# yutongwangBIT/multi_orbslam3

Hardware: AMD Instinct MI355X
Metric: tracking+localBA frames/sec (aggregate over agents; 1 agent per GPU) (higher is better)
Workload: dtype u8/int32 (ORB front-end, Hamming), f64 (local BA)

## Files before the change

multi_orbslam3_amd/csrc/lba.hip:

```cpp

#include <time.h>

#include <condition_variable>
#include <atomic>
#include <unistd.h>
#include <mutex>
#include <thread>

#include "common.hpp"
#include "wave.hpp"

#include <algorithm>
#include <cmath>
#include <limits>
#include <numeric>
#include <type_traits>

using namespace orbg;

#include "ldlt_mfma.hpp"
#include "ldlt_xcd.hpp"
#include "se3.hpp"
#include "lm_driver.hpp"

// ... 544 lines not shown
                                               const double* __restrict__ points, CamT c, Huber hb, double* __restrict__ err,
                                               double* __restrict__ chi2, const int* __restrict__ pose_col,
                                               const int* __restrict__ point_col, double* __restrict__ EB,
                                               const int* __restrict__ ps_start, const int* __restrict__ ps_edges,
                                               double* __restrict__ Hpp, double* __restrict__ bp, double* __restrict__ partial,
                                               unsigned* __restrict__ ticket, const double* __restrict__ scale_partial, int n_scale_partial,
                                               const int* __restrict__ ok_flag, HostRec* __restrict__ rec, unsigned seq, int n_edge_blocks,
                                               int nL, const int* __restrict__ pt_start, const int* __restrict__ pt_edges,
                                               double* __restrict__ Hll, double* __restrict__ bl, LmIn lm) {
  const int bid = (int)blockIdx.x;
  LBA_PROF_BEGIN(0);
  if (bid < nP) {
    lin_poses_block<true>(bid, ps_start, ps_edges, edges, poses, points, c, hb, err, chi2, Hpp, bp);
  } else if (bid < nP + n_edge_blocks) {
    linearize_block<true>(bid - nP, n_edges, edges, poses, points, c, hb, err, chi2, pose_col, point_col, EB,
                          TrialPublish{partial, ticket, scale_partial, n_scale_partial, ok_flag, rec, seq, n_edge_blocks, lm});
  } else if (bid - nP - n_edge_blocks < errlin_point_blocks(nL)) {
    lin_points_block(bid - nP - n_edge_blocks, nL, pt_start, pt_edges, edges, poses, points, c, hb, Hll, bl);
  } else {
    publish_trial_when_all_arrived(n_edge_blocks, partial, ticket, scale_partial, n_scale_partial, ok_flag, rec, seq, lm);
  }
  LBA_PROF_END();
}


__global__ __launch_bounds__(256) void k_reduce_points(int nL, const int* __restrict__ pt_start, const int* __restrict__ pt_edges,
                                                      const double* __restrict__ EB, double* __restrict__ Hll, double* __restrict__ bl) {
  const int l = blockIdx.x * 256 + threadIdx.x;
  if (l >= nL) return;
  double acc[9];
#pragma unroll
  for (int i = 0; i < 9; i++) acc[i] = 0;
  const int jb = pt_start[l], je = pt_start[l + 1];
  double part[4][9];
#pragma unroll
  for (int q = 0; q < 4; q++)
#pragma unroll
    for (int i = 0; i < 9; i++) part[q][i] = 0;
  for (int j0 = jb; j0 < je; j0 += 4) {
    int id[4];
#pragma unroll
    for (int q = 0; q < 4; q++) id[q] = pt_edges[min(j0 + q, je - 1)];
    double v[4][9];
#pragma unroll
    for (int q = 0; q < 4; q++) {
      const double* eb = EB + (size_t)id[q] * kEB + 18;
#pragma unroll
      for (int i = 0; i < 9; i++) v[q][i] = eb[i];
    }
#pragma unroll
    for (int q = 0; q < 4; q++)
      if (j0 + q < je) {
#pragma unroll
        for (int i = 0; i < 9; i++) part[q][i] += v[q][i];
      }
  }
#pragma unroll
  for (int i = 0; i < 9; i++) acc[i] = ((part[0][i] + part[1][i]) + part[2][i]) + part[3][i];
  for (int i = 0; i < 6; i++) Hll[6 * (size_t)l + i] = acc[i];
  for (int i = 0; i < 3; i++) bl[3 * (size_t)l + i] = acc[6 + i];
}

__device__ inline void inv3_sym(const double* h6, double lambda, double* o) {
  const double m0 = h6[0] + lambda, m1 = h6[1], m2 = h6[2], m4 = h6[3] + lambda, m5 = h6[4], m8 = h6[5] + lambda;
  const double c00 = m4 * m8 - m5 * m5, c01 = m5 * m2 - m1 * m8, c02 = m1 * m5 - m4 * m2;
  const double det = m0 * c00 + m1 * c01 + m2 * c02;
  const double id = 1.0 / det;
  o[0] = c00 * id; o[1] = c01 * id; o[2] = c02 * id;
  o[3] = o[1]; o[4] = (m0 * m8 - m2 * m2) * id; o[5] = (m2 * m1 - m0 * m5) * id;
  o[6] = o[2]; o[7] = o[5]; o[8] = (m0 * m4 - m1 * m1) * id;
}

struct PairItem { int ea, eb, l; };

constexpr int kSchurThreads = 256;

constexpr int kSortPfThreads = 64, kSortPfCap = 64;
template <int NT, int CAP, bool BY_EDGE = false>
__device__ __forceinline__ void sort_pf_block(int bid, int nL, const int* __restrict__ pf_start, int* __restrict__ pf_edges,
                                              int* __restrict__ pf_col, unsigned long long* __restrict__ lm_mask,
                                              const lba_edge* __restrict__ edges, const int* __restrict__ pose_col) {
  __shared__ int s_e[NT][CAP + 1];
  __shared__ int s_c[NT][CAP + 1];
  const int l = bid * NT + threadIdx.x;
  if (l >= nL) return;
  const int b0 = pf_start[l], cnt = pf_start[l + 1] - b0;
  unsigned long long m = 0;
  if (cnt <= CAP) {
    int* const se = s_e[threadIdx.x];
    int* const sc = s_c[threadIdx.x];
    for (int j = 0; j < cnt; j++) se[j] = pf_edges[b0 + j];
    for (int j = 0; j < cnt; j++) sc[j] = pose_col[edges[se[j]].pose];
    for (int a2 = 1; a2 < cnt; a2++) {
      const int e = se[a2], key = sc[a2];
      int b2 = a2 - 1;
      while (b2 >= 0 && (sc[b2] > key || (BY_EDGE && sc[b2] == key && se[b2] > e))) { se[b2 + 1] = se[b2]; sc[b2 + 1] = sc[b2]; b2--; }
      se[b2 + 1] = e; sc[b2 + 1] = key;
    }
    for (int j = 0; j < cnt; j++) { pf_edges[b0 + j] = se[j]; pf_col[b0 + j] = sc[j]; m |= 1ull << sc[j]; }
  } else {
    for (int a2 = b0 + 1; a2 < b0 + cnt; a2++) {
      const int e = pf_edges[a2], key = pose_col[edges[e].pose];
      int b2 = a2 - 1;
      while (b2 >= b0 && (pose_col[edges[pf_edges[b2]].pose] > key ||
                          (BY_EDGE && pose_col[edges[pf_edges[b2]].pose] == key && pf_edges[b2] > e))) { pf_edges[b2 + 1] = pf_edges[b2]; b2--; }
      pf_edges[b2 + 1] = e;
    }
    for (int j = b0; j < b0 + cnt; j++) { const int c = pose_col[edges[pf_edges[j]].pose]; pf_col[j] = c; m |= 1ull << c; }
  }
  lm_mask[l] = m;
}

__global__ __launch_bounds__(256) void k_csr_fill(int n_edges, const lba_edge* __restrict__ edges, const int* __restrict__ pose_col,
                                                 const int* __restrict__ point_col, int* __restrict__ cur_pt, int* __restrict__ cur_ps,
                                                 int* __restrict__ cur_pf, int* __restrict__ pt_edges, int* __restrict__ ps_edges,
                                                 int* __restrict__ pf_edges) {
  __shared__ int s_cnt[64], s_base[64];
  const int k = blockIdx.x * 256 + threadIdx.x;
  if (threadIdx.x < 64) s_cnt[threadIdx.x] = 0;
  __syncthreads();
  int lc = -1, pc = -1, my = 0;
  if (k < n_edges) {
    const lba_edge e = edges[k];
    lc = point_col[e.point]; pc = pose_col[e.pose];
    pt_edges[atomicAdd(&cur_pt[lc], 1)] = k;
    if (pc >= 0) { pf_edges[atomicAdd(&cur_pf[lc], 1)] = k; my = atomicAdd(&s_cnt[pc], 1); }
  }
  __syncthreads();
  if (threadIdx.x < 64 && s_cnt[threadIdx.x] > 0) s_base[threadIdx.x] = atomicAdd(&cur_ps[threadIdx.x], s_cnt[threadIdx.x]);
  __syncthreads();
  if (pc >= 0) ps_edges[s_base[pc] + my] = k;
}
constexpr int kPrep256Cap = 16, kPrep256Pad = 8, kPrep256Zero = 4;
constexpr int kCsrPoseCap = 4096, kCsrPtCap = 16;
__global__ __launch_bounds__(256) void k_csr_sort(int nP, int nL, const int* __restrict__ ps_start, int* __restrict__ ps_edges,
                                                 const int* __restrict__ pt_start, int* __restrict__ pt_edges,
                                                 const int* __restrict__ pf_start, int* __restrict__ pf_edges, int* __restrict__ pf_col,
                                                 unsigned long long* __restrict__ lm_mask, const lba_edge* __restrict__ edges,
                                                 const int* __restrict__ pose_col, int n_unknowns, double* __restrict__ St,
                                                 double* __restrict__ xzero, int n_zero) {
  __shared__ int s_pose[kCsrPoseCap];
  __shared__ int s_pt[256][kCsrPtCap + 1];
  int bid = (int)blockIdx.x;
  const int tid = threadIdx.x;
  if (bid < nP) {
    const int b0 = ps_start[bid], cnt = ps_start[bid + 1] - b0;
    int m = 1;
    while (m < cnt) m <<= 1;
    for (int i = tid; i < m; i += 256) s_pose[i] = i < cnt ? ps_edges[b0 + i] : 0x7FFFFFFF;
    __syncthreads();
    for (int k2 = 2; k2 <= m; k2 <<= 1)
      for (int j = k2 >> 1; j > 0; j >>= 1) {
        for (int i = tid; i < m; i += 256) {
          const int ixj = i ^ j;
          if (ixj > i) {
            const int a = s_pose[i], c = s_pose[ixj];
            const bool up = (i & k2) == 0;
            if ((a > c) == up) { s_pose[i] = c; s_pose[ixj] = a; }
          }
        }
        __syncthreads();
      }
    for (int i = tid; i < cnt; i += 256) ps_edges[b0 + i] = s_pose[i];
    return;
  }
  bid -= nP;
  const int n_pt_blocks = (nL + 255) / 256;
  if (bid < n_pt_blocks) {
    const int l = bid * 256 + tid;
    if (l < nL) {
      const int b0 = pt_start[l], cnt = pt_start[l + 1] - b0;
      if (cnt <= kCsrPtCap) {
        int* const se = s_pt[tid];
        for (int j = 0; j < cnt; j++) se[j] = pt_edges[b0 + j];
        for (int a2 = 1; a2 < cnt; a2++) {
          const int e = se[a2];
          int b2 = a2 - 1;
          while (b2 >= 0 && se[b2] > e) { se[b2 + 1] = se[b2]; b2--; }
          se[b2 + 1] = e;
        }
        for (int j = 0; j < cnt; j++) pt_edges[b0 + j] = se[j];
      } else {
        for (int a2 = b0 + 1; a2 < b0 + cnt; a2++) {
          const int e = pt_edges[a2];
          int b2 = a2 - 1;
          while (b2 >= b0 && pt_edges[b2] > e) { pt_edges[b2 + 1] = pt_edges[b2]; b2--; }
          pt_edges[b2 + 1] = e;
        }
      }
    }
    sort_pf_block<256, kCsrPtCap, true>(bid, nL, pf_start, pf_edges, pf_col, lm_mask, edges, pose_col);
    return;
  }
  bid -= n_pt_blocks;
  if (bid < kPrep256Pad) { if (St) ldltm::image_pad_range(n_unknowns, St, bid * 256 + tid, kPrep256Pad * 256); return; }
  bid -= kPrep256Pad;
  for (int i = bid * 256 + tid; i < n_zero; i += kPrep256Zero * 256) xzero[i] = 0.0;
}

template <class CamT>
__global__ __launch_bounds__(256) void k_errlin_prep(int n_errlin_blocks, int n_sort_blocks, int* __restrict__ pf_edges_w, int* __restrict__ pf_col_w,
                                                    const int* __restrict__ pf_start, unsigned long long* __restrict__ lm_mask,
                                                    int n_unknowns, double* __restrict__ St, double* __restrict__ xzero, int n_zero,
                                                    int nP, int n_edges, const lba_edge* __restrict__ edges, const PoseQ* __restrict__ poses,
                                               const double* __restrict__ points, CamT c, Huber hb, double* __restrict__ err,
                                               double* __restrict__ chi2, const int* __restrict__ pose_col,
                                               const int* __restrict__ point_col, double* __restrict__ EB,
                                               const int* __restrict__ ps_start, const int* __restrict__ ps_edges,
                                               double* __restrict__ Hpp, double* __restrict__ bp, double* __restrict__ partial,
                                               unsigned* __restrict__ ticket, const double* __restrict__ scale_partial, int n_scale_partial,
                                               const int* __restrict__ ok_flag, HostRec* __restrict__ rec, unsigned seq, int n_edge_blocks,
                                               int nL, const int* __restrict__ pt_start, const int* __restrict__ pt_edges,
                                               double* __restrict__ Hll, double* __restrict__ bl, LmIn lm) {
  int bid = (int)blockIdx.x;
  if (bid >= n_errlin_blocks) {
    bid -= n_errlin_blocks;
    if (bid < n_sort_blocks) { sort_pf_block<256, kPrep256Cap>(bid, nL, pf_start, pf_edges_w, pf_col_w, lm_mask, edges, pose_col); return; }
    bid -= n_sort_blocks;
    if (bid < kPrep256Pad) { if (St) ldltm::image_pad_range(n_unknowns, St, bid * 256 + (int)threadIdx.x, kPrep256Pad * 256); return; }
    bid -= kPrep256Pad;
    for (int i = bid * 256 + (int)threadIdx.x; i < n_zero; i += kPrep256Zero * 256) xzero[i] = 0.0;
    return;
  }

  
  if (bid < nP) {
    lin_poses_block<true>(bid, ps_start, ps_edges, edges, poses, points, c, hb, err, chi2, Hpp, bp);
  } else if (bid < nP + n_edge_blocks) {
    linearize_block<true>(bid - nP, n_edges, edges, poses, points, c, hb, err, chi2, pose_col, point_col, EB,
                          TrialPublish{partial, ticket, scale_partial, n_scale_partial, ok_flag, rec, seq, n_edge_blocks, lm});
  } else if (bid - nP - n_edge_blocks < errlin_point_blocks(nL)) {
    lin_points_block(bid - nP - n_edge_blocks, nL, pt_start, pt_edges, edges, poses, points, c, hb, Hll, bl);
  } else {
    publish_trial_when_all_arrived(n_edge_blocks, partial, ticket, scale_partial, n_scale_partial, ok_flag, rec, seq, lm);
  }
}

__global__ __launch_bounds__(kSortPfThreads) void k_prep(int n_sort_blocks, int nL, const int* __restrict__ pf_start, int* __restrict__ pf_edges,
                                                        int* __restrict__ pf_col, unsigned long long* __restrict__ lm_mask,
                                                        const lba_edge* __restrict__ edges, const int* __restrict__ pose_col,
                                                        int n, double* __restrict__ St, double* __restrict__ xzero, int n_zero) {
  constexpr int kPadBlocks = 32;
  const int bid = (int)blockIdx.x;
  if (bid < n_sort_blocks) { sort_pf_block<kSortPfThreads, kSortPfCap>(bid, nL, pf_start, pf_edges, pf_col, lm_mask, edges, pose_col); return; }
  if (bid < n_sort_blocks + kPadBlocks) {
    if (St) ldltm::image_pad_range(n, St, (bid - n_sort_blocks) * kSortPfThreads + (int)threadIdx.x, kPadBlocks * kSortPfThreads);
    return;
  }
  const int nz = (int)gridDim.x - n_sort_blocks - kPadBlocks;
  for (int i = (bid - n_sort_blocks - kPadBlocks) * kSortPfThreads + (int)threadIdx.x; i < n_zero; i += nz * kSortPfThreads) xzero[i] = 0.0;
}

__device__ __forceinline__ void build_items_block(int pr, int nP, int nL, const unsigned long long* __restrict__ lm_mask,
                                                  const int* __restrict__ pf_start, const int* __restrict__ pf_edges,
                                                  const int* __restrict__ pf_col, PairItem* __restrict__ items, int cap,
                                                  int* __restrict__ pair_count) {
  __shared__ int wcount[4];
  const int tid = threadIdx.x, lane = tid & 63, wv = tid >> 6;
  int i1 = 0, rem = pr;
  while (rem >= nP - i1) { rem -= nP - i1; i1++; }
  const int i2 = i1 + rem;
  const unsigned long long need = (1ull << i1) | (1ull << i2);
  PairItem* out = items + (size_t)pr * cap;
  int running = 0;
  for (int l0 = 0; l0 < nL; l0 += 256) {
    const int l = l0 + tid;
    const unsigned long long m = l < nL ? lm_mask[l] : 0ull;
    const bool has = (m & need) == need;
    const unsigned long long bal = __ballot(has);
    if (lane == 0) wcount[wv] = __popcll(bal);
    __syncthreads();
    int before = 0, total = 0;
#pragma unroll
    for (int w = 0; w < 4; w++) { const int c = wcount[w]; if (w < wv) before += c; total += c; }
    if (has) {
      const int pos = running + before + __popcll(bal & ((1ull << lane) - 1ull));
      const int b0 = pf_start[l];
      const int ea = pf_edges[b0 + __popcll(m & ((1ull << i1) - 1ull))];
      const int eb = pf_edges[b0 + __popcll(m & ((1ull << i2) - 1ull))];
      if (pos < cap) out[pos] = PairItem{ea, eb, l};
    }
    running += total;
    __syncthreads();
  }
  if (tid == 0) pair_count[pr] = min(running, cap);
}
__global__ __launch_bounds__(256) void k_build_items(int nP, int nL, const unsigned long long* __restrict__ lm_mask,
                                                    const int* __restrict__ pf_start, const int* __restrict__ pf_edges,
                                                    const int* __restrict__ pf_col, PairItem* __restrict__ items, int cap,
                                                    int* __restrict__ pair_count) {
  build_items_block((int)blockIdx.x, nP, nL, lm_mask, pf_start, pf_edges, pf_col, items, cap, pair_count);
}

template <int PASSES>
__global__ __launch_bounds__(kSchurThreads) void k_schur(int nP, const int* __restrict__ pair_i1, const int* __restrict__ pair_i2,
                                                        const int* __restrict__ pair_start, const PairItem* __restrict__ items,
                                                        const double* __restrict__ EB, const double* __restrict__ Hll,
                                                        const double* __restrict__ bl, const double* __restrict__ Hpp,
                                                        const double* __restrict__ bp, double lambda_v, double* __restrict__ S,
                                                        double* __restrict__ bs, const double* __restrict__ lambda_p, int item_cap,
                                                        const int* __restrict__ pair_count, double* __restrict__ St) {
  const double lambda = lambda_p ? *lambda_p : lambda_v;
  constexpr int kSeg = 65, kRow = 4 * kSeg + 1, kPass = 42 / PASSES;
  __shared__ double red[kPass * kRow];
  __shared__ double part[42][4];
  LBA_PROF_BEGIN(1);
  int pr;
  {
    const int nb = gridDim.x, q = nb >> 3, r = nb & 7, k = blockIdx.x & 7;
    pr = k * q + min(k, r) + (blockIdx.x >> 3);
  }
  int i1, i2;
  if (pair_i1) { i1 = pair_i1[pr]; i2 = pair_i2[pr]; }
  else {
    int rem = pr; i1 = 0;
    while (rem >= nP - i1) { rem -= nP - i1; i1++; }
    i2 = i1 + rem;
  }
  const int tid = threadIdx.x;
  double acc[36], cacc[6];
#pragma unroll
  for (int i = 0; i < 36; i++) acc[i] = 0;
#pragma unroll
  for (int i = 0; i < 6; i++) cacc[i] = 0;
  const bool diag = i1 == i2;
  const int j0 = pair_start ? pair_start[pr] : pr * item_cap;
  const int j1 = pair_start ? pair_start[pr + 1] : j0 + pair_count[pr];
  for (int j = j0 + tid; j < j1; j += kSchurThreads) {
    const PairItem it = items[j];
    double Dinv[9];
    inv3_sym(Hll + 6 * (size_t)it.l, lambda, Dinv);
    const double* Bi = EB + (size_t)it.ea * kEB;
    const double* Bj = EB + (size_t)it.eb * kEB;
    double BD[18];
#pragma unroll
    for (int a = 0; a < 6; a++)
#pragma unroll
      for (int c = 0; c < 3; c++) BD[3 * a + c] = Bi[3 * a] * Dinv[c] + Bi[3 * a + 1] * Dinv[3 + c] + Bi[3 * a + 2] * Dinv[6 + c];
#pragma unroll
    for (int a = 0; a < 6; a++)
#pragma unroll
      for (int c = 0; c < 6; c++) acc[6 * a + c] += BD[3 * a] * Bj[3 * c] + BD[3 * a + 1] * Bj[3 * c + 1] + BD[3 * a + 2] * Bj[3 * c + 2];
    if (diag) {
      const double* b = bl + 3 * (size_t)it.l;
#pragma unroll
      for (int a = 0; a < 6; a++) cacc[a] += BD[3 * a] * b[0] + BD[3 * a + 1] * b[1] + BD[3 * a + 2] * b[2];
    }
  }
  LBA_PROF_PHASE(0, 0);
  const int slot = (tid >> 6) * kSeg + (tid & 63);
  const int nval = diag ? 42 : 36;
#pragma unroll
  for (int ps = 0; ps < PASSES; ps++) {
    if (ps == 1) __syncthreads();
#pragma unroll
    for (int i = 0; i < kPass; i++) {
      const int v = ps * kPass + i;
      red[i * kRow + slot] = v < 36 ? acc[v < 36 ? v : 0] : cacc[v >= 36 ? v - 36 : 0];
    }
    __syncthreads();
    if (tid < 4 * kPass && ps * kPass + (tid >> 2) < nval) {
      const int o = tid >> 2, q = tid & 3;
      const double* r = red + o * kRow + q * kSeg;
      double s = 0;
#pragma unroll
      for (int k0 = 0; k0 < 64; k0 += 16) {
        double v[16];
#pragma unroll
        for (int u = 0; u < 16; u++) v[u] = r[k0 + u];
#pragma unroll
        for (int u = 0; u < 16; u++) s += v[u];
      }
      part[ps * kPass + o][q] = s;
    }
  }
  __syncthreads();
  LBA_PROF_PHASE(0, 1);
  const int n = 6 * nP;
  if (tid < 36) {
    const double s = ((part[tid][0] + part[tid][1]) + part[tid][2]) + part[tid][3];
    const int a = tid / 6, c = tid % 6;
    double v = -s;
    if (diag) {
      const int lo = a < c ? a : c, hi = a < c ? c : a;
      const int u = lo * 6 - lo * (lo - 1) / 2 + (hi - lo);
      v += Hpp[21 * (size_t)i1 + u] + (a == c ? lambda : 0.0);
    }
    if (St) {
      const int r = 6 * i1 + a, cc = 6 * i2 + c;
      const int p0 = ldltm::tile_image_pos(r, cc), p1 = ldltm::tile_image_pos(cc, r);
      if (p0 >= 0) St[p0] = v;
      if (p1 >= 0 && r != cc) St[p1] = v;
    } else {
      S[(size_t)(6 * i1 + a) * n + 6 * i2 + c] = v;
      if (!diag) S[(size_t)(6 * i2 + c) * n + 6 * i1 + a] = v;
    }
  } else if (diag && tid < 42) {
    const int a = tid - 36;
    const double s = ((part[tid][0] + part[tid][1]) + part[tid][2]) + part[tid][3];
    const double v = bp[6 * (size_t)i1 + a] - s;
    bs[6 * i1 + a] = v;
    if (St) ldltm::image_put_rhs(St, n, 6 * i1 + a, v);
  }
  LBA_PROF_END();
}

#include "ldlt_wide.hpp"

template <int NT>
__global__ __launch_bounds__(NT) void k_update(int n_poses, int n_points, int nP, const int* __restrict__ pose_col,
                                               const int* __restrict__ point_col, const PoseQ* __restrict__ poses,
                                               const double* __restrict__ points, double* __restrict__ x,
                                               const int* __restrict__ pf_start, const int* __restrict__ pf_edges,
                                               const int* __restrict__ pf_col, const double* __restrict__ EB,
                                               const double* __restrict__ Hll, const double* __restrict__ bl, double lambda_v,
                                               PoseQ* __restrict__ poses_out, double* __restrict__ points_out,
                                               const double* __restrict__ bp, double* __restrict__ scale_partial,
                                               const double* __restrict__ lambda_p) {
  LBA_PROF_BEGIN(2);
  const double lambda = lambda_p ? *lambda_p : lambda_v;
  __shared__ double red[NT];
  const int i = blockIdx.x * NT + threadIdx.x;
  double sc = 0;
  if (i < n_points) {
    const int l = point_col[i];
    double dx[3] = {0, 0, 0};
    if (l >= 0) {
      double cl[3] = {bl[3 * (size_t)l], bl[3 * (size_t)l + 1], bl[3 * (size_t)l + 2]};
      constexpr int kUpdChunk = 8;
      const int j1 = pf_start[l + 1];
      for (int j0 = pf_start[l]; j0 < j1; j0 += kUpdChunk) {
        int eid[kUpdChunk], col[kUpdChunk];
#pragma unroll
        for (int u = 0; u < kUpdChunk; u++) { const int j = min(j0 + u, j1 - 1); eid[u] = pf_edges[j]; col[u] = pf_col[j]; }
        double Bv[kUpdChunk][18], xv[kUpdChunk][6];
#pragma unroll
        for (int u = 0; u < kUpdChunk; u++) {
          const double* Bi = EB + (size_t)eid[u] * kEB;
          const double* xp = x + 6 * (size_t)col[u];
#pragma unroll
          for (int q = 0; q < 18; q++) Bv[u][q] = Bi[q];
#pragma unroll
          for (int a = 0; a < 6; a++) xv[u][a] = xp[a];
        }
#pragma unroll
        for (int u = 0; u < kUpdChunk; u++)
          if (j0 + u < j1) {
#pragma unroll
            for (int c = 0; c < 3; c++)
#pragma unroll
              for (int a = 0; a < 6; a++) cl[c] -= Bv[u][3 * a + c] * xv[u][a];
          }
      }
      double Dinv[9];
      inv3_sym(Hll + 6 * (size_t)l, lambda, Dinv);
      for (int a = 0; a < 3; a++) {
        dx[a] = Dinv[3 * a] * cl[0] + Dinv[3 * a + 1] * cl[1] + Dinv[3 * a + 2] * cl[2];
        x[6 * (size_t)nP + 3 * (size_t)l + a] = dx[a];
        sc += dx[a] * (lambda * dx[a] + bl[3 * (size_t)l + a]);
      }
    }
    for (int a = 0; a < 3; a++) points_out[3 * (size_t)i + a] = points[3 * (size_t)i + a] + dx[a];
  } else if (i < n_points + n_poses) {
    const int p = i - n_points;
    const int c = pose_col[p];
    if (c >= 0) {
      pose_oplus(poses[p], x + 6 * (size_t)c, &poses_out[p]);
      for (int a = 0; a < 6; a++) { const double xv = x[6 * (size_t)c + a]; sc += xv * (lambda * xv + bp[6 * (size_t)c + a]); }
    } else {
      poses_out[p] = poses[p];
    }
  }
  LBA_PROF_PHASE(0, 0);
  red[threadIdx.x] = sc;
  __syncthreads();
  for (int s2 = NT / 2; s2 > 0; s2 >>= 1) {
    if ((int)threadIdx.x < s2) red[threadIdx.x] += red[threadIdx.x + s2];
    __syncthreads();
  }
  if (threadIdx.x == 0) scale_partial[blockIdx.x] = red[0];
  LBA_PROF_END();
}

__device__ __forceinline__ void finish_block(int n_partial, const double* __restrict__ partial, int nP, int nL,
                                             const double* __restrict__ x, const double* __restrict__ bp, const double* __restrict__ bl,
                                             const double* __restrict__ Hpp, const double* __restrict__ Hll, double lambda,
                                             const int* __restrict__ ok_flag, int want_scale, int want_maxdiag, HostRec* __restrict__ rec,
                                             double lambda_init, double* __restrict__ lambda0_out) {
  __shared__ double red[256];
  __shared__ double parts[1024];
  const int tid = threadIdx.x;
  for (int i = tid; i < n_partial && i < 1024; i += 256) parts[i] = partial[i];
  __syncthreads();
  double chi = 0;
  if (tid == 0) {
    const int nl = min(n_partial, 1024);
    int i = 0;
    for (; i + 16 <= nl; i += 16) {
      double v[16];
#pragma unroll
      for (int u = 0; u < 16; u++) v[u] = parts[i + u];
#pragma unroll
      for (int u = 0; u < 16; u++) chi += v[u];
    }
    for (; i < nl; i++) chi += parts[i];
    for (i = 1024; i < n_partial; i++) chi += partial[i];
  }
  double sc = 0;
  if (want_scale) {
    const int n6 = 6 * nP, n3 = 3 * nL;
    for (int j = tid; j < n6; j += 256) sc += x[j] * (lambda * x[j] + bp[j]);
    for (int j = tid; j < n3; j += 256) sc += x[n6 + j] * (lambda * x[n6 + j] + bl[j]);
  }
  red[tid] = sc;
  __syncthreads();
  for (int s = 128; s > 0; s >>= 1) {
    if (tid < s) red[tid] += red[tid + s];
    __syncthreads();
  }
  const double scale = red[0];
  __syncthreads();
  double mx = 0;
  if (want_maxdiag) {
    for (int i = tid; i < nP; i += 256) {
      const double* h = Hpp + 21 * (size_t)i;
      const int di[6] = {0, 6, 11, 15, 18, 20};
      for (int j = 0; j < 6; j++) mx = fmax(mx, fabs(h[di[j]]));
    }
    for (int i = tid; i < nL; i += 256) {
      const double* h = Hll + 6 * (size_t)i;
      mx = fmax(mx, fmax(fabs(h[0]), fmax(fabs(h[3]), fabs(h[5]))));
    }
  }
  red[tid] = mx;
  __syncthreads();
  for (int s = 128; s > 0; s >>= 1) {
    if (tid < s) red[tid] = fmax(red[tid], red[tid + s]);
    __syncthreads();
  }
  if (tid == 0) {
    if (lambda0_out) {
      rec->chi2_init = chi; rec->maxdiag = red[0];
      lambda0_out[0] = lambda_init > 0 ? lambda_init : 1e-5 * red[0];
      lambda0_out[2] = chi;
    } else {
      rec->chi2 = chi; rec->scale = scale; rec->maxdiag = red[0]; rec->ok = ok_flag ? *ok_flag : 1;
    }
  }
}
__global__ __launch_bounds__(256) void k_finish(int n_partial, const double* __restrict__ partial, int nP, int nL,
                                               const double* __restrict__ x, const double* __restrict__ bp, const double* __restrict__ bl,
                                               const double* __restrict__ Hpp, const double* __restrict__ Hll, double lambda,
                                               const int* __restrict__ ok_flag, int want_scale, int want_maxdiag, HostRec* __restrict__ rec,
                                               double lambda_init, double* __restrict__ lambda0_out) {
  finish_block(n_partial, partial, nP, nL, x, bp, bl, Hpp, Hll, lambda, ok_flag, want_scale, want_maxdiag, rec, lambda_init, lambda0_out);
}
__global__ __launch_bounds__(256) void k_finish_items(int n_partial, const double* __restrict__ partial, int nP, int nL,
                                                     const double* __restrict__ bp, const double* __restrict__ bl,
                                                     const double* __restrict__ Hpp, const double* __restrict__ Hll, HostRec* __restrict__ rec,
                                                     double lambda_init, double* __restrict__ lambda0_out,
                                                     const unsigned long long* __restrict__ lm_mask, const int* __restrict__ pf_start,
                                                     const int* __restrict__ pf_edges, const int* __restrict__ pf_col,
                                                     PairItem* __restrict__ items, int cap, int* __restrict__ pair_count) {
  if (blockIdx.x == 0)
    finish_block(n_partial, partial, nP, nL, nullptr, bp, bl, Hpp, Hll, 0.0, nullptr, 0, 1, rec, lambda_init, lambda0_out);
  else
    build_items_block((int)blockIdx.x - 1, nP, nL, lm_mask, pf_start, pf_edges, pf_col, items, cap, pair_count);
}

}


struct LbaSwitches {
  bool ldlt_wide = false;
  int ldlt_xcd = 1;
  bool ldlt_xcd_short_once = false;
  static LbaSwitches from_env() {
    LbaSwitches w;
    w.ldlt_wide = getenv("ORBG_LDLT_WIDE") != nullptr;
    if (const char* e = getenv("ORBG_LDLT_XCD")) { w.ldlt_xcd = !strcmp(e, "0") ? 0 : !strcmp(e, "safe") ? 2 : 1; w.ldlt_xcd_short_once = !strcmp(e, "short"); }
    return w;
  }
};
struct LinSet {
  DevBuf<double> EB, Hll, bl, Hpp, bp;
  int reserve(int NE, int nL, int nP) {
    int rc;
    if ((rc = EB.reserve(std::max<size_t>((size_t)NE * kEB, 1))) || (rc = Hll.reserve(std::max<size_t>(6 * (size_t)nL, 1))) ||
        (rc = bl.reserve(std::max<size_t>(3 * (size_t)nL, 1))) || (rc = Hpp.reserve(std::max<size_t>(21 * (size_t)nP, 1))) ||
        (rc = bp.reserve(std::max<size_t>(6 * (size_t)nP, 1))))
      return rc;
    return ORBG_OK;
  }
  void release() { EB.release(); Hll.release(); bl.release(); Hpp.release(); bp.release(); }
};
struct lba_handle {
  int device = 0;
  hipStream_t stream = nullptr;
  bool ext_stream = false;
  LbaSwitches sw;
  ldltm::AttrCache ldlt_attr;
  ldltx::Context ldlt_x;
  long long xcd_timeouts = 0;
  DevBuf<double> d_xscr;
  DevBuf<unsigned> d_xflags;
  DevBuf<lba_edge> d_edges;
  PinnedBuf<lba_edge> edges_pin;
  DevBuf<PairItem> d_items_dev;
  DevBuf<int> d_pair_count;
  DevBuf<PoseQ> d_poses[2];
  DevBuf<double> d_points[2];
  DevBuf<double> d_err, d_chi2, d_partial, d_S, d_bs, d_x;
  LinSet lin[2];
  DevBuf<double> d_lambda0;
  DevBuf<double> d_wide;
  DevBuf<double> d_St, d_wfac;
  DevBuf<int> d_ok;
  PinnedBuf<HostRec> rec;
  unsigned rec_seq = 0;
  PinnedBuf<uint8_t> up_h, dl_h;
  DevBuf<uint8_t> up_d;
  DevBuf<double> d_scale_partial;
  DevBuf<unsigned> d_ticket;
  StreamSignal sig;
  std::vector<int> s_pose_deg, s_point_deg, s_pose_col, s_point_col, s_pf_deg, s_f1, s_f2, s_f3, s_fill, s_row_off, s_junk;
  std::vector<unsigned> s_cnt4;
  int prof_on = 0;
  hipEvent_t prof_ev[2] = {nullptr, nullptr};
  double prof_sum_ms = 0; long long prof_n = 0; int prof_n_unknowns = 0;
  long long prof_solves = 0;
  std::thread worker;
  std::mutex mu;
  std::condition_variable cv;
  std::atomic<bool> quit{false};
  std::atomic<int> job_state{0};
  const lba_problem* job_p = nullptr; StopRef job_stop; lba_result* job_r = nullptr;
  int job_status = ORBG_OK;
  double job_ms = 0;
};

extern "C" int lba_create(int device, int cap_poses, int cap_points, int cap_edges, lba_handle** out) {
  if (!out || cap_poses < 0 || cap_points < 0 || cap_edges < 0) return ORBG_BAD_ARG;
  int rc = select_device(device);
  if (rc) return rc;
  lba_handle* h = new lba_handle();
  h->device = device;
  h->sw = LbaSwitches::from_env();
  if (orbg::create_stream(&h->stream, "lba") != hipSuccess) { delete h; return ORBG_HIP_ERROR; }
  if ((rc = h->rec.reserve(4)) || (rc = h->d_ok.reserve(4))) { delete h; return rc; }
  memset(h->rec.h, 0, 4 * sizeof(HostRec));
  (void)cap_poses; (void)cap_points; (void)cap_edges;
  *out = h;
  return ORBG_OK;
}

extern "C" int lba_set_stream(lba_handle* h, void* hip_stream) {
  if (!h) return ORBG_BAD_ARG;
  if (h->job_state.load() != 0) return ORBG_BAD_ARG;
  int rc = select_device(h->device);
  if (rc) return rc;
  return orbg::swap_stream(&h->stream, &h->ext_stream, hip_stream, "lba");
}

extern "C" int lba_destroy(lba_handle* h) {
  if (!h) return ORBG_BAD_ARG;
  if (h->worker.joinable()) {
    { std::lock_guard<std::mutex> lk(h->mu); h->quit = true; }
    h->cv.notify_all();
    h->worker.join();
  }
  (void)hipSetDevice(h->device);
  (void)hipStreamSynchronize(h->stream);
  h->d_xscr.release(); h->d_xflags.release(); h->ldlt_x.scr = nullptr; h->ldlt_x.flags = nullptr;
  h->d_edges.release(); h->edges_pin.release(); h->d_items_dev.release(); h->d_pair_count.release();
  for (int i = 0; i < 2; i++) { h->d_poses[i].release(); h->d_points[i].release(); }
  h->d_err.release(); h->d_chi2.release(); h->d_partial.release(); h->d_S.release(); h->d_bs.release(); h->d_x.release();
  for (LinSet& L : h->lin) L.release();
  h->d_lambda0.release(); h->d_wide.release(); h->d_St.release(); h->d_wfac.release(); h->d_ok.release(); h->rec.release();
  h->up_h.release(); h->dl_h.release(); h->up_d.release(); h->d_scale_partial.release(); h->d_ticket.release(); h->sig.release();
  for (auto& e : h->prof_ev) if (e) { (void)hipEventDestroy(e); e = nullptr; }
  if (!h->ext_stream) orbg::release_stream(h->stream);
  delete h;
  return ORBG_OK;
}

struct TraceAcc {
  double t[8] = {0}; long n = 0; const char* name;
  explicit TraceAcc(const char* nm) : name(nm) {}
  ~TraceAcc() {
    if (n && getenv("ORBG_TRACE")) {
      fprintf(stderr, "[orbgpu trace] %s n=%ld:", name, n);
      for (int i = 0; i < 8; i++) fprintf(stderr, " %.1f", t[i] / n * 1e6);
      fprintf(stderr, " us\n");
    }
  }
};
static inline double now_s() { timespec ts; clock_gettime(CLOCK_MONOTONIC, &ts); return ts.tv_sec + 1e-9 * ts.tv_nsec; }

__global__ __launch_bounds__(256) void k_upload16(const uint4* __restrict__ src, uint4* __restrict__ dst, unsigned n16) {
  const unsigned i = blockIdx.x * 256u + threadIdx.x;
  if (i < n16) dst[i] = src[i];
}
static void upload16(const uint8_t* src, uint8_t* dst, size_t bytes, hipStream_t st) {
// ... 892 lines not shown
```

Before: 8952.

## Exploit symmetry and batch loads for diagonal Schur blocks

Diagonal pose-pair blocks in the Schur kernel now accumulate only the 21 upper-triangular entries, since Bi equals Bj there, and reduce 27 values instead of 42. The diagonal path loads several items per thread ahead of compute, with asm barriers to force register staging and overlap memory latency. Off-diagonal items are also staged in registers when PASSES is 1. The Hpp/bp prefetch is hoisted before the loop. The cost is higher register pressure, which may lower occupancy.

```diff
diff --git a/multi_orbslam3_amd/csrc/lba.hip b/multi_orbslam3_amd/csrc/lba.hip
--- a/multi_orbslam3_amd/csrc/lba.hip
+++ b/multi_orbslam3_amd/csrc/lba.hip
@@ -870,6 +870,7 @@
                                                         const int* __restrict__ pair_count, double* __restrict__ St) {
   const double lambda = lambda_p ? *lambda_p : lambda_v;
   constexpr int kSeg = 65, kRow = 4 * kSeg + 1, kPass = 42 / PASSES;
+  constexpr int kRounds = PASSES == 1 ? 3 : 1;
   __shared__ double red[kPass * kRow];
   __shared__ double part[42][4];
   LBA_PROF_BEGIN(1);
@@ -894,37 +895,106 @@
   const bool diag = i1 == i2;
   const int j0 = pair_start ? pair_start[pr] : pr * item_cap;
   const int j1 = pair_start ? pair_start[pr + 1] : j0 + pair_count[pr];
-  for (int j = j0 + tid; j < j1; j += kSchurThreads) {
-    const PairItem it = items[j];
-    double Dinv[9];
-    inv3_sym(Hll + 6 * (size_t)it.l, lambda, Dinv);
-    const double* Bi = EB + (size_t)it.ea * kEB;
-    const double* Bj = EB + (size_t)it.eb * kEB;
-    double BD[18];
-#pragma unroll
-    for (int a = 0; a < 6; a++)
-#pragma unroll
-      for (int c = 0; c < 3; c++) BD[3 * a + c] = Bi[3 * a] * Dinv[c] + Bi[3 * a + 1] * Dinv[3 + c] + Bi[3 * a + 2] * Dinv[6 + c];
-#pragma unroll
-    for (int a = 0; a < 6; a++)
-#pragma unroll
-      for (int c = 0; c < 6; c++) acc[6 * a + c] += BD[3 * a] * Bj[3 * c] + BD[3 * a + 1] * Bj[3 * c + 1] + BD[3 * a + 2] * Bj[3 * c + 2];
-    if (diag) {
-      const double* b = bl + 3 * (size_t)it.l;
-#pragma unroll
-      for (int a = 0; a < 6; a++) cacc[a] += BD[3 * a] * b[0] + BD[3 * a + 1] * b[1] + BD[3 * a + 2] * b[2];
+  double hpre = 0;
+  if (diag) {
+    const int a = tid / 6, c = tid % 6, lo = a < c ? a : c, hi = a < c ? c : a;
+    hpre = *(tid < 36 ? Hpp + 21 * (size_t)i1 + (lo * 6 - lo * (lo - 1) / 2 + (hi - lo)) : bp + 6 * (size_t)i1 + min(tid - 36, 5));
+    for (int g0 = j0; g0 < j1; g0 += kRounds * kSchurThreads) {
+      PairItem it[kRounds];
+#pragma unroll
+      for (int r = 0; r < kRounds; r++) it[r] = items[min(g0 + r * kSchurThreads + tid, j1 - 1)];
+      double Hv[kRounds][6], Bv[kRounds][18], bv[kRounds][3];
+#pragma unroll
+      for (int r = 0; r < kRounds; r++) {
+        const double* h = Hll + 6 * (size_t)it[r].l;
+        const double* Bi = EB + (size_t)it[r].ea * kEB;
+        const double* b = bl + 3 * (size_t)it[r].l;
+#pragma unroll
+        for (int q = 0; q < 6; q++) Hv[r][q] = h[q];
+#pragma unroll
+        for (int q = 0; q < 18; q++) Bv[r][q] = Bi[q];
+#pragma unroll
+        for (int q = 0; q < 3; q++) bv[r][q] = b[q];
+      }
+#pragma unroll
+      for (int r = 0; r < kRounds; r++) {
+#pragma unroll
+        for (int q = 0; q < 6; q++) asm volatile("" : "+v"(Hv[r][q]));
+#pragma unroll
+        for (int q = 0; q < 18; q++) asm volatile("" : "+v"(Bv[r][q]));
+#pragma unroll
+        for (int q = 0; q < 3; q++) asm volatile("" : "+v"(bv[r][q]));
+        if (g0 + r * kSchurThreads + tid < j1) {
+          double Dinv[9];
+          inv3_sym(Hv[r], lambda, Dinv);
+          const double* Bi = Bv[r];
+          const double* Bj = Bv[r];
+          double BD[18];
+#pragma unroll
+          for (int a = 0; a < 6; a++)
+#pragma unroll
+            for (int c = 0; c < 3; c++) BD[3 * a + c] = Bi[3 * a] * Dinv[c] + Bi[3 * a + 1] * Dinv[3 + c] + Bi[3 * a + 2] * Dinv[6 + c];
+#pragma unroll
+          for (int a = 0; a < 6; a++)
+#pragma unroll
+            for (int c = a; c < 6; c++)
+              acc[a * 6 - a * (a - 1) / 2 + (c - a)] += BD[3 * a] * Bj[3 * c] + BD[3 * a + 1] * Bj[3 * c + 1] + BD[3 * a + 2] * Bj[3 * c + 2];
+          const double* b = bv[r];
+#pragma unroll
+          for (int a = 0; a < 6; a++) cacc[a] += BD[3 * a] * b[0] + BD[3 * a + 1] * b[1] + BD[3 * a + 2] * b[2];
+        }
+      }
+    }
+    asm volatile("" : "+v"(hpre));
+  } else {
+    for (int j = j0 + tid; j < j1; j += kSchurThreads) {
+      const PairItem it = items[j];
+      const double* Hl = Hll + 6 * (size_t)it.l;
+      const double* Bi = EB + (size_t)it.ea * kEB;
+      const double* Bj = EB + (size_t)it.eb * kEB;
+      double Hv[6], Bvi[18], Bvj[18];
+      if constexpr (PASSES == 1) {
+#pragma unroll
+        for (int q = 0; q < 6; q++) Hv[q] = Hl[q];
+#pragma unroll
+        for (int q = 0; q < 18; q++) { Bvi[q] = Bi[q]; Bvj[q] = Bj[q]; }
+#pragma unroll
+        for (int q = 0; q < 6; q++) asm volatile("" : "+v"(Hv[q]));
+#pragma unroll
+        for (int q = 0; q < 18; q++) { asm volatile("" : "+v"(Bvi[q])); asm volatile("" : "+v"(Bvj[q])); }
+        Hl = Hv; Bi = Bvi; Bj = Bvj;
+      }
+      double Dinv[9];
+      inv3_sym(Hl, lambda, Dinv);
+      double BD[18];
+#pragma unroll
+      for (int a = 0; a < 6; a++)
+#pragma unroll
+        for (int c = 0; c < 3; c++) BD[3 * a + c] = Bi[3 * a] * Dinv[c] + Bi[3 * a + 1] * Dinv[3 + c] + Bi[3 * a + 2] * Dinv[6 + c];
+#pragma unroll
+      for (int a = 0; a < 6; a++)
+#pragma unroll
+        for (int c = 0; c < 6; c++) acc[6 * a + c] += BD[3 * a] * Bj[3 * c] + BD[3 * a + 1] * Bj[3 * c + 1] + BD[3 * a + 2] * Bj[3 * c + 2];
     }
   }
   LBA_PROF_PHASE(0, 0);
   const int slot = (tid >> 6) * kSeg + (tid & 63);
-  const int nval = diag ? 42 : 36;
+  const int nval = diag ? 27 : 36;
 #pragma unroll
   for (int ps = 0; ps < PASSES; ps++) {
     if (ps == 1) __syncthreads();
-#pragma unroll
-    for (int i = 0; i < kPass; i++) {
-      const int v = ps * kPass + i;
-      red[i * kRow + slot] = v < 36 ? acc[v < 36 ? v : 0] : cacc[v >= 36 ? v - 36 : 0];
+    if (diag) {
+#pragma unroll
+      for (int i = 0; i < kPass; i++) {
+        const int v = ps * kPass + i;
+        if (v < 27) red[i * kRow + slot] = v < 21 ? acc[v < 21 ? v : 0] : cacc[v >= 21 ? v - 21 : 0];
+      }
+    } else {
+#pragma unroll
+      for (int i = 0; i < kPass; i++) {
+        const int v = ps * kPass + i;
+        red[i * kRow + slot] = v < 36 ? acc[v < 36 ? v : 0] : cacc[v >= 36 ? v - 36 : 0];
+      }
     }
     __syncthreads();
     if (tid < 4 * kPass && ps * kPass + (tid >> 2) < nval) {
@@ -946,14 +1016,12 @@
   LBA_PROF_PHASE(0, 1);
   const int n = 6 * nP;
   if (tid < 36) {
-    const double s = ((part[tid][0] + part[tid][1]) + part[tid][2]) + part[tid][3];
     const int a = tid / 6, c = tid % 6;
+    const int lo = a < c ? a : c, hi = a < c ? c : a;
+    const int w = diag ? lo * 6 - lo * (lo - 1) / 2 + (hi - lo) : tid;
+    const double s = ((part[w][0] + part[w][1]) + part[w][2]) + part[w][3];
     double v = -s;
-    if (diag) {
-      const int lo = a < c ? a : c, hi = a < c ? c : a;
-      const int u = lo * 6 - lo * (lo - 1) / 2 + (hi - lo);
-      v += Hpp[21 * (size_t)i1 + u] + (a == c ? lambda : 0.0);
-    }
+    if (diag) v += hpre + (a == c ? lambda : 0.0);
     if (St) {
       const int r = 6 * i1 + a, cc = 6 * i2 + c;
       const int p0 = ldltm::tile_image_pos(r, cc), p1 = ldltm::tile_image_pos(cc, r);
@@ -965,8 +1033,8 @@
     }
   } else if (diag && tid < 42) {
     const int a = tid - 36;
-    const double s = ((part[tid][0] + part[tid][1]) + part[tid][2]) + part[tid][3];
-    const double v = bp[6 * (size_t)i1 + a] - s;
+    const double s = ((part[21 + a][0] + part[21 + a][1]) + part[21 + a][2]) + part[21 + a][3];
+    const double v = hpre - s;
     bs[6 * i1 + a] = v;
     if (St) ldltm::image_put_rhs(St, n, 6 * i1 + a, v);
   }
```

Measured after the change: 8853. 0.989x the previous value.
